# handasontam/PERT-GNN-KDD23

Measured on AMD Instinct MI355X. Metric: training graphs/sec (whole node), higher is better.
Workload: dtype bf16; 1 GPU; model=PERT-GNN 8L/256H, global_batch=1024, vocab=realistic, interfaces=2041, entry_unions=266, graph_mode=full, parallelism=dp1

## Files before the change

### csrc/bindings.cpp

```cpp
#include <hip/hip_runtime.h>
#include <torch/extension.h>

#include <climits>
#include <cstdlib>
#include <memory>
#include <optional>
#include <string>
#include <vector>

#include <c10/cuda/CUDAStream.h>

#include "hip/attn_bn.h"
#include "hip/gemm_dispatch.h"

namespace {

#define CHECK_IN(t)                                                      \
  TORCH_CHECK((t).is_cuda(), #t " must be on GPU");                      \
  TORCH_CHECK((t).is_contiguous(), #t " must be contiguous")

inline hipStream_t cur_stream() {
  return (hipStream_t)c10::cuda::getCurrentCUDAStream().stream();
}

// ... 143 lines not shown
                 float, float, float, float, hipStream_t);
void launch_adam_dynamic(float*, const float*, float*, float*, float*, float*,
                         long, float, float, float, float, float, float,
                         float, hipStream_t);
void launch_gemm_f32_nt(const float*, const float*, const float*, float*, int,
                        int, int, bool, hipStream_t);
void launch_gemm_f32_nn(const float*, const float*, const float*, float*, int,
                        int, int, bool, hipStream_t);
void launch_gemm_f32_tn(const float*, const float*, float*, float*, int, int,
                        int, hipStream_t);
void launch_colsum(const float*, float*, long, int, hipStream_t);
void launch_gemm_bf16_nt(const float*, const float*, const float*, float*,
                         int, int, int, bool, hipStream_t);
void launch_gemm_bf16_nn(const float*, const float*, const float*, float*,
                         int, int, int, bool, hipStream_t);
void launch_gemm_bf16_tn(const float*, const float*, float*, float*, int, int,
                         int, hipStream_t);
void launch_gemm_fp16_nt(const float*, const float*, const float*, float*,
                         int, int, int, bool, hipStream_t);
void launch_gemm_fp16_nn(const float*, const float*, const float*, float*,
                         int, int, int, bool, hipStream_t);
void launch_gemm_fp16_tn(const float*, const float*, float*, float*, int, int,
                         int, hipStream_t);
void launch_embed_grouped_scatter(const float*, const int*, const int*, float*,
                                  float*, long, int, int, int, int, int,
                                  hipStream_t);
void launch_embed_grouped_scatter_bal(const void*, int, const int*,
                                      const int*, const int*, const int*,
                                      const int*, const int*, float*, float*,
                                      float*, int, int, int, int, int, int,
                                      hipStream_t);
void launch_rows_sum_lists(const void*, int, const int*, const int*, void*, int,
                           int, int, int, hipStream_t);
void launch_vocab_scatter(const float*, const long*, long, float*, long, int,
                          int, int, int, hipStream_t);
void launch_vocab_scatter_dual(const float*, const long*, int, float*, float*,
                               long, int, int, int, hipStream_t);
void launch_edge_attn_fused_fwd(const float*, const float*, const float*,
                                const long*, int, const int*, const int*,
                                float*, float*, int, int, int, hipStream_t);
void launch_edge_attn_fused_bwd(const float*, const float*, const float*,
                                const float*, const long*, int, const float*,
                                const int*, const int*, const int*,
                                const int*, const int*, float*, float*,
                                float*, int, int, long, int, hipStream_t);
void launch_edge_attn_fused_fwd16(const void*, const void*, const void*,
                                  int, const long*, int, const int*,
                                  const int*, void*, int, float*, int, int,
                                  int, hipStream_t);
void launch_edge_attn_fused_bwd16(const void*, int, const void*,
                                  const void*, const void*, int, const long*,
                                  int, const float*, const int*, const int*,
                                  const int*, const int*, const int*, void*,
                                  void*, float*, int, int, long, int,
                                  hipStream_t, const AttnBnBwd* = nullptr,
                                  const AttnPoolBwd* = nullptr);
void launch_bn_bwd_partials_affine16(const void*, const void*,
                                     const unsigned char*, const float*,
                                     const float*, long, int, float*, float,
                                     float*, float*, float*, hipStream_t,
                                     bool acc = false);
void launch_edge_attn_fused_infer(const float*, const float*, const float*,
                                  const long*, int, const int*, const int*,
                                  const float*, const float*, int, float*,
                                  int, int, int, hipStream_t);
void launch_edge_attn_fused_infer16(const void*, const void*, const void*,
// ... 559 lines not shown
              "out_dtype must be bf16 or fp32");
  for (const auto& t : {idx1, lptr1, idx2, lptr2, idx3, lptr3})
    TORCH_CHECK(t.scalar_type() == torch::kInt32 && t.dim() == 1,
                "plan tensors must be 1-D int32");
  TORCH_CHECK(V >= 0 && R >= 0 && lptr3.numel() == V + R + 1,
              "lptr3 must have V+R+1 entries");
  TORCH_CHECK(lptr1.numel() >= 1 && lptr2.numel() >= 1,
              "lptr1/lptr2 must have at least one entry");
  TORCH_CHECK(idx1.numel() == de.size(0),
              "level 1 must list every row of de exactly once");
  const int h = (int)de.size(1);
  const long n1 = lptr1.numel() - 1;
  const long n2 = lptr2.numel() - 1;
  const int in16 = de.scalar_type() == torch::kBFloat16 ? 1 : 0;
  const int out16 = out_dtype == torch::kBFloat16 ? 1 : 0;
  auto partial =
      torch::empty({n1 + n2, (long)h}, de.options().dtype(torch::kFloat32));
  auto out = torch::empty({V + R, (long)h}, de.options().dtype(out_dtype));
  hipStream_t s = cur_stream();
  launch_rows_sum_lists(de.data_ptr(), in16, idx1.data_ptr<int>(),
                        lptr1.data_ptr<int>(), partial.data_ptr(), 0, (int)n1,
                        h, (int)unroll, s);
  if (n2 > 0)
    launch_rows_sum_lists(partial.data_ptr(), 0, idx2.data_ptr<int>(),
                          lptr2.data_ptr<int>(),
                          partial.data_ptr<float>() + n1 * h, 0, (int)n2, h,
                          (int)unroll, s);
  launch_rows_sum_lists(partial.data_ptr(), 0, idx3.data_ptr<int>(),
                        lptr3.data_ptr<int>(), out.data_ptr(), out16,
                        (int)(V + R), h, (int)unroll, s);
  return out;
}

std::vector<torch::Tensor> edge_attn_fused_fwd(
    torch::Tensor qkvs, torch::Tensor pifc, torch::Tensor prpc,
    torch::Tensor ea, torch::Tensor row_ptr, torch::Tensor csr_src,
    bool out16, int64_t heads = 1) {
  CHECK_IN(qkvs); CHECK_IN(pifc); CHECK_IN(prpc); CHECK_IN(ea);
  const int n = qkvs.size(0);
  const int h = qkvs.size(1) / 4;
  TORCH_CHECK(h <= 512, "H must be <= 512");
  TORCH_CHECK(heads >= 1 && heads <= h && h % heads == 0,
              "heads must divide H (H=", h, ", heads=", heads, ")");
  auto fopt = qkvs.options().dtype(torch::kFloat32);
  const bool b16 = qkvs.scalar_type() == torch::kBFloat16;
  const bool p16 = pifc.scalar_type() == torch::kBFloat16;
  TORCH_CHECK(!out16 || b16, "out16 requires bf16 qkvs");
  TORCH_CHECK(!p16 || b16, "bf16 P tables require bf16 qkvs");
  TORCH_CHECK(pifc.scalar_type() == prpc.scalar_type(),
              "P tables must share a dtype");
  auto out = torch::empty({n, h}, out16 ? qkvs.options() : fopt);
  auto alpha = heads == 1 ? torch::empty({ea.size(0)}, fopt)
                          : torch::empty({ea.size(0), heads}, fopt);
  if (b16) {
    launch_edge_attn_fused_fwd16(
        qkvs.data_ptr(), pifc.data_ptr(), prpc.data_ptr(), p16 ? 1 : 0,
        ea.data_ptr<long>(), (int)ea.size(1),
        row_ptr.data_ptr<int>(), csr_src.data_ptr<int>(),
        out.data_ptr(), out16 ? 1 : 0, alpha.data_ptr<float>(), n, h,
        (int)heads, cur_stream());
  } else {
    launch_edge_attn_fused_fwd(
        qkvs.data_ptr<float>(), pifc.data_ptr<float>(), prpc.data_ptr<float>(),
        ea.data_ptr<long>(), (int)ea.size(1), row_ptr.data_ptr<int>(),
        csr_src.data_ptr<int>(), out.data_ptr<float>(), alpha.data_ptr<float>(),
        n, h, (int)heads, cur_stream());
// ... 1087 lines not shown
                    sink_t[1] ? sink_t[1] : d_rpc.data_ptr<float>()};
  const int ms[2] = {(int)rows[0], (int)rows[1]};
  const bool addto[2] = {sink_t[0] != nullptr || splits > 1,
                         sink_t[1] != nullptr || splits > 1};
  launch_ptables_dgrad(dp_d.data(), w_d.data(), npairs, outs, ms, h, splits,
                       addto, s);
  launch_ptables_wgrad((int)dp_w.size(), dp_w.data(), a_w.data(), dw_w.data(),
                       m_w.data(), h, false, s, sunk.get());
  return {d_ifc, d_rpc, dW};
}

PYBIND11_MODULE(TORCH_EXTENSION_NAME, mod) {
  mod.def("ptables_fwd", &ptables_fwd, py::arg("ifc_table"),
          py::arg("rpc_table"), py::arg("we_ifc"), py::arg("we_rpc"));
  mod.def("ptables_bwd", &ptables_bwd, py::arg("dP"), py::arg("ifc_table"),
          py::arg("rpc_table"), py::arg("we_ifc"), py::arg("we_rpc"),
          py::arg("dgrad_splits") = 1, py::arg("d_ifc_sink") = py::none(),
          py::arg("d_rpc_sink") = py::none(),
          py::arg("dw_sinks") = std::vector<OptTensor>());
  mod.def("ptables_max_groups", &ptables_max_groups);
  mod.def("linear_fwd_bf16_o16", &linear_fwd_bf16_o16);
  mod.def("linear_dgrad16", &linear_dgrad16);
  mod.def("linear_wgrad16", &linear_wgrad16, py::arg("g"), py::arg("x"),
          py::arg("has_bias"), py::arg("dw_sink") = py::none(),
          py::arg("db_sink") = py::none(), py::arg("tile") = 0);
  mod.def("vocab_scatter_dual", &vocab_scatter_dual);
  mod.def("linear_dgrad", &linear_dgrad);
  mod.def("linear_wgrad", &linear_wgrad);
  mod.def("embed_grouped_scatter_bal", &embed_grouped_scatter_bal);
  mod.def("edge_table_grad", &edge_table_grad, py::arg("de"), py::arg("idx1"),
          py::arg("lptr1"), py::arg("idx2"), py::arg("lptr2"),
          py::arg("idx3"), py::arg("lptr3"), py::arg("V"), py::arg("R"),
          py::arg("out_dtype"), py::arg("unroll") = 8);
  mod.def("bn_stats", &bn_stats);
  mod.def("bn_finalize_apply", &bn_finalize_apply, py::arg("x"),
          py::arg("partials"), py::arg("gamma"), py::arg("beta"),
          py::arg("running_mean"), py::arg("running_var"), py::arg("momentum"),
          py::arg("eps"), py::arg("training"), py::arg("relu"),
          py::arg("dropout_p") = 0.0, py::arg("seed") = torch::Tensor());
  mod.def("bn_bwd_partials", &bn_bwd_partials, py::arg("g"), py::arg("x"),
          py::arg("y"), py::arg("mean"), py::arg("invstd"), py::arg("relu"),
          py::arg("keep_inv") = 1.0);
  mod.def("bn_bwd_apply", &bn_bwd_apply, py::arg("g"), py::arg("x"),
          py::arg("y"), py::arg("mean"), py::arg("invstd"), py::arg("gamma"),
          py::arg("partials_global"), py::arg("partials_local"),
          py::arg("relu"), py::arg("keep_inv") = 1.0,
          py::arg("dgamma_sink") = py::none(),
          py::arg("dbeta_sink") = py::none());
  mod.def("vocab_scatter", &vocab_scatter);
  mod.def("collate_native", &collate_native,
          py::call_guard<py::gil_scoped_release>());
  mod.def("edge_attn_fused_fwd", &edge_attn_fused_fwd, py::arg("qkvs"),
          py::arg("pifc"), py::arg("prpc"), py::arg("edge_attr"),
          py::arg("row_ptr"), py::arg("csr_src"), py::arg("out16"),
          py::arg("heads") = 1);
  mod.def("edge_attn_fused_bwd", &edge_attn_fused_bwd, py::arg("g"),
          py::arg("qkvs"), py::arg("pifc"), py::arg("prpc"),
          py::arg("edge_attr"), py::arg("alpha"), py::arg("row_ptr"),
          py::arg("csr_src"), py::arg("col_ptr"), py::arg("csc_dst"),
          py::arg("csc_eid"), py::arg("heads") = 1);
  mod.def("edge_attn_fused_infer", &edge_attn_fused_infer, py::arg("qkvs"),
          py::arg("pifc"), py::arg("prpc"), py::arg("edge_attr"),
          py::arg("row_ptr"), py::arg("csr_src"), py::arg("bn_scale"),
          py::arg("bn_shift"), py::arg("relu"), py::arg("out16"),
          py::arg("heads") = 1);
  mod.def("embed_grouped_scatter", &embed_grouped_scatter);
// ... 99 lines not shown
```

### csrc/hip/gemm.hip

```cpp

#include "common.h"
#include "gemm_dispatch.h"
#include <cstdlib>

static inline bool pertgnn_deterministic() {
  const char* e = getenv("PERTGNN_DETERMINISTIC");
  return e && e[0] == '1';
}

#define GEMM_BK 32
#define GEMM_THREADS 256

typedef __attribute__((ext_vector_type(4))) float f32x4;


template <int BF>
__device__ __forceinline__ void stage_transpose(
    const float* __restrict__ g, long ld, int free0, int contract0,
    int free_max, int contract_max, float* lds) {
  const int t = threadIdx.x;
  const int fr = t / 8;
  const int cq = (t % 8) * 4;
  const bool interior = (free0 + BF <= free_max) &&
                        (contract0 + GEMM_BK <= contract_max);
// ... 319 lines not shown
        a, b, bias, c, m, n, k2, relu ? 1 : 0);
  } else {
    const int grid = ((m + 63) / 64) * ((k2 + 63) / 64);
    gemm_f32_nn_kernel<64, 64><<<dim3(grid), dim3(GEMM_THREADS), 0, s>>>(
        a, b, bias, c, m, n, k2, relu ? 1 : 0);
  }
}

void launch_gemm_f32_tn(const float* a, const float* b, float* c, float* dbias,
                        int m, int n, int k2, hipStream_t s) {
  const bool big = gemm_dispatch::tn_tile128(n, k2);
  const int tiles = gemm_dispatch::tn_tiles(n, k2);
  const int slices =
      gemm_dispatch::tn_slices(m, tiles, GEMM_BK, pertgnn_deterministic());
  if (slices > 1)
    HIP_CHECK(hipMemsetAsync(c, 0, (long)n * k2 * sizeof(float), s));
  if (dbias) HIP_CHECK(hipMemsetAsync(dbias, 0, n * sizeof(float), s));
  if (big)
    gemm_f32_tn_kernel<128, 128>
        <<<dim3(tiles * slices), dim3(GEMM_THREADS), 0, s>>>(a, b, c, dbias, m,
                                                             n, k2, slices);
  else
    gemm_f32_tn_kernel<64, 64>
        <<<dim3(tiles * slices), dim3(GEMM_THREADS), 0, s>>>(a, b, c, dbias, m,
                                                             n, k2, slices);
}

void launch_colsum(const float* g, float* out, long m, int n, hipStream_t s) {
  HIP_CHECK(hipMemsetAsync(out, 0, n * sizeof(float), s));
  const int blocks = (int)min((long)256, (m + 63) / 64);
  colsum_par_kernel<<<dim3(blocks), dim3(256), n * sizeof(float), s>>>(g, out,
                                                                       m, n);
}
```

### csrc/hip/segops.hip

```cpp
#include "common.h"
#include <cstdlib>


#define WAVES_PER_BLOCK 4

template <int VPT, typename TX = float>
__global__ void seg_pool_p1_kernel(const TX* __restrict__ x,
                                   const float* __restrict__ probs,
                                   const float* __restrict__ nn,
                                   const int* __restrict__ batch_ptr,
                                   float* __restrict__ partial, int b, int P,
                                   int h) {
  const int wid = threadIdx.x / PERTGNN_WAVE;
  const int lane = threadIdx.x % PERTGNN_WAVE;
  const int w = blockIdx.x * WAVES_PER_BLOCK + wid;
  if (w >= b * P) return;
  const int g = w / P;
  const int sub = w % P;
  float acc[VPT];
#pragma unroll
  for (int j = 0; j < VPT; ++j) acc[j] = 0.f;
  for (int i = batch_ptr[g] + sub; i < batch_ptr[g + 1]; i += P) {
    const float wt = probs[i] / nn[i];
#pragma unroll
// ... 371 lines not shown
    embed_grouped_p2_kernel<V>                                                 \
        <<<dim3(ceil_div(rows, WAVES_PER_BLOCK)), block, 0, s>>>(              \
            partial, dtable, rows, P, h);                                      \
    break;
    CASE(1) CASE(2) CASE(3) CASE(4) CASE(5) CASE(6) CASE(7) CASE(8)
#undef CASE
    default: pertgnn_shape_fail("segops launcher", "vpt", vpt);
  }
}

template <int VPT, typename T>
__device__ __forceinline__ void rows_sum_load(const T* __restrict__ row,
                                              int lane, float (&v)[VPT]) {
  if constexpr (sizeof(T) == 2) {
#pragma unroll
    for (int q = 0; q < VPT; q += 4) {
      const segb4 x = *reinterpret_cast<const segb4*>(
          (const __bf16*)row + lane * VPT + q);
#pragma unroll
      for (int u = 0; u < 4; ++u) v[q + u] = (float)x[u];
    }
  } else {
#pragma unroll
    for (int q = 0; q < VPT; q += 4) {
      const segf4 x = *reinterpret_cast<const segf4*>(
          (const float*)row + lane * VPT + q);
#pragma unroll
      for (int u = 0; u < 4; ++u) v[q + u] = x[u];
    }
  }
}

template <int VPT, typename TIn, typename TOut, int U>
__global__ void rows_sum_lists_kernel(const TIn* __restrict__ src,
                                      const int* __restrict__ idx,
                                      const int* __restrict__ lptr,
                                      TOut* __restrict__ out, int n_lists) {
  static_assert(VPT % 4 == 0, "packed loads need 4 columns per lane");
  constexpr int H = VPT * PERTGNN_WAVE;
  const int lane = threadIdx.x % PERTGNN_WAVE;
  const int w = __builtin_amdgcn_readfirstlane(
      blockIdx.x * WAVES_PER_BLOCK + threadIdx.x / PERTGNN_WAVE);
  if (w >= n_lists) return;
  const int p0 = lptr[w];
  const int p1 = lptr[w + 1];
  float acc[VPT];
#pragma unroll
  for (int j = 0; j < VPT; ++j) acc[j] = 0.f;
  int p = p0;
  for (; p + U <= p1; p += U) {
    int r[U];
#pragma unroll
    for (int u = 0; u < U; ++u) r[u] = idx[p + u];
    float v[U][VPT];
#pragma unroll
    for (int u = 0; u < U; ++u)
      rows_sum_load<VPT>(src + (long)r[u] * H, lane, v[u]);
#pragma unroll
    for (int u = 0; u < U; ++u)
#pragma unroll
      for (int j = 0; j < VPT; ++j) acc[j] += v[u][j];
  }
  if (p < p1) {
    int r[U];
#pragma unroll
    for (int u = 0; u < U; ++u) r[u] = idx[min(p + u, p1 - 1)];
    float v[U][VPT];
#pragma unroll
    for (int u = 0; u < U; ++u)
      rows_sum_load<VPT>(src + (long)r[u] * H, lane, v[u]);
#pragma unroll
    for (int u = 0; u < U; ++u)
      if (p + u < p1) {
#pragma unroll
        for (int j = 0; j < VPT; ++j) acc[j] += v[u][j];
      }
  }
  TOut* dst = out + (long)w * H + lane * VPT;
  if constexpr (sizeof(TOut) == 2) {
#pragma unroll
    for (int q = 0; q < VPT; q += 4) {
      segb4 o;
#pragma unroll
      for (int u = 0; u < 4; ++u) o[u] = (__bf16)acc[q + u];
      *reinterpret_cast<segb4*>((__bf16*)dst + q) = o;
    }
  } else {
#pragma unroll
    for (int q = 0; q < VPT; q += 4) {
      segf4 o;
#pragma unroll
      for (int u = 0; u < 4; ++u) o[u] = acc[q + u];
      *reinterpret_cast<segf4*>((float*)dst + q) = o;
    }
  }
}

void launch_rows_sum_lists(const void* src, int in16, const int* idx,
                           const int* lptr, void* out, int out16, int n_lists,
                           int h, int unroll, hipStream_t s) {
  if (n_lists == 0) return;
  if (h != 256 && h != 512) pertgnn_shape_fail("rows_sum_lists", "h", h);
  if (unroll != 4 && unroll != 8)
    pertgnn_shape_fail("rows_sum_lists", "unroll", unroll);
  if (in16 && out16) pertgnn_shape_fail("rows_sum_lists", "in16+out16", 1);
  const dim3 block(WAVES_PER_BLOCK * PERTGNN_WAVE);
  const dim3 grid(ceil_div(n_lists, WAVES_PER_BLOCK));
#define RSL(V, TI, TO, UU)                                                     \
  rows_sum_lists_kernel<V, TI, TO, UU><<<grid, block, 0, s>>>(                 \
      (const TI*)src, idx, lptr, (TO*)out, n_lists)
#define RSL_T(V, UU)                                                           \
  do {                                                                         \
    if (in16) RSL(V, __bf16, float, UU);                                       \
    else if (out16) RSL(V, float, __bf16, UU);                                 \
    else RSL(V, float, float, UU);                                             \
  } while (0)
  if (h == 256) {
    if (unroll == 8) RSL_T(4, 8); else RSL_T(4, 4);
  } else {
    if (unroll == 8) RSL_T(8, 8); else RSL_T(8, 4);
  }
#undef RSL_T
#undef RSL
}

__global__ void vocab_scatter_kernel(const float* __restrict__ g,
                                     const long* __restrict__ idx,
                                     long idx_stride, float* __restrict__ dtable,
                                     long n, int rows, int h, int gstride,
                                     int col_off) {
  extern __shared__ float acc[];
  const long vh = (long)rows * h;
  for (long t = threadIdx.x; t < vh; t += blockDim.x) acc[t] = 0.f;
  __syncthreads();
  const int wid = threadIdx.x / PERTGNN_WAVE;
  const int lane = threadIdx.x % PERTGNN_WAVE;
  const long rows_per_block = (n + gridDim.x - 1) / gridDim.x;
  const long r0 = (long)blockIdx.x * rows_per_block;
  const long r1 = min(n, r0 + rows_per_block);
  for (long r = r0 + wid; r < r1; r += WAVES_PER_BLOCK) {
    const long v = idx[r * idx_stride];
    for (int c = lane; c < h; c += PERTGNN_WAVE)
      atomicAdd(&acc[v * h + c], g[r * gstride + col_off + c]);
  }
  __syncthreads();
  for (long t = threadIdx.x; t < vh; t += blockDim.x)
    if (acc[t] != 0.f) atomicAdd(&dtable[t], acc[t]);
}

__global__ void vocab_scatter_vec_kernel(const float* __restrict__ g,
                                         const long* __restrict__ idx,
                                         long idx_stride,
                                         float* __restrict__ dtable, long n,
                                         int rows, int h, int gstride,
                                         int col_off) {
  typedef __attribute__((ext_vector_type(4))) float f4;
// ... 1775 lines not shown
```

### pertgnn/models/pert_gnn.py

```python
from __future__ import annotations

import torch
import torch.nn.functional as F
from torch import nn

from ..ops import functional as ops


class _EdgeLinearView:

    def __init__(self, conv):
        object.__setattr__(self, "_conv", conv)

    @property
    def weight(self):
        c = self._conv
        return torch.cat([c.we_ifc, c.we_rpc], dim=1)

    bias = None


class _SegLinearView:

    def __init__(self, conv, seg, has_bias=True):
# ... 123 lines not shown

    def forward_fused(self, x, edge_attr, ifc_weight, rpc_weight, csr,
                      out16=False, pifc=None, prpc=None):
        qkvs, pifc, prpc = self._fused_operands(x, ifc_weight, rpc_weight,
                                                pifc, prpc)
        return ops.edge_attention_fused(qkvs, pifc, prpc, edge_attr, csr,
                                        out16=out16, heads=self.heads)

    def forward_fused_bn(self, x, edge_attr, ifc_weight, rpc_weight, csr, bn,
                         comm=None, dropout_p=0.0, pifc=None, prpc=None):
        qkvs, pifc, prpc = self._fused_operands(x, ifc_weight, rpc_weight,
                                                pifc, prpc)
        return ops.edge_attention_fused_bn_relu(
            qkvs, pifc, prpc, edge_attr, csr, bn.weight, bn.bias,
            bn.running_mean, bn.running_var, bn.momentum, bn.eps,
            heads=self.heads, comm=comm, dropout_p=dropout_p)

    def forward_fused_pool(self, x, edge_attr, ifc_weight, rpc_weight, csr,
                           probs, nnodes, batch, num_graphs, pifc=None,
                           prpc=None):
        qkvs, pifc, prpc = self._fused_operands(x, ifc_weight, rpc_weight,
                                                pifc, prpc)
        return ops.edge_attention_fused_pool(
            qkvs, pifc, prpc, edge_attr, csr, probs, nnodes, batch,
            num_graphs, heads=self.heads)

    def _fused_operands(self, x, ifc_weight, rpc_weight, pifc, prpc):
        h = self.out_channels
        if x.shape[1] != self.k_padded:
            x = torch.nn.functional.pad(x, (0, self.k_padded - x.shape[1]))
        act16 = (ops.gemm_precision() in ("bf16", "fp16") and h % 256 == 0
                 and ops.act16_enabled())
        if act16:
            qkvs = ops.linear16(x, self.w4, self.b4)
            if pifc is not None and prpc is not None:
                pass
            elif ops.p16_enabled():
                pifc = ops.linear16(ifc_weight, self.we_ifc)
                prpc = ops.linear16(rpc_weight, self.we_rpc)
            else:
                pifc = ops.linear(ifc_weight, self.we_ifc, None)
                prpc = ops.linear(rpc_weight, self.we_rpc, None)
        else:
            qkvs = ops.linear(x, self.w4, self.b4)
            pifc = ops.linear(ifc_weight, self.we_ifc, None)
            prpc = ops.linear(rpc_weight, self.we_rpc, None)
        return qkvs, pifc, prpc


class SAGEDeterministic(nn.Module):

    def __init__(
        self,
        in_channels,
        cat_dims,
        entry_id_max,
        interface_id_max,
        rpctype_id_max,
        hidden_channels,
        num_layers,
        dropout,
        *,
        heads=1,
    ):
        super().__init__()
        self.heads = heads
        self.convs = nn.ModuleList()
# ... 140 lines not shown
```

### pertgnn/ops/functional.py

```python
from __future__ import annotations

from typing import NamedTuple

import torch

from . import reference as ref
from .backend import ext, use_hip


def deterministic() -> bool:
    import os
    return os.environ.get("PERTGNN_DETERMINISTIC", "0") == "1"


def grad_sink(p):
    sink = getattr(p, "_grad_sink", None)
    if sink is None or not p.requires_grad or not torch.is_grad_enabled():
        return None
    import os
    if os.environ.get("PERTGNN_NO_GRAD_SINK", "0") == "1":
        return None
    g = p.grad
    if g is None or g.data_ptr() != sink.data_ptr() or g.shape != sink.shape:
        return None
# ... 160 lines not shown
    assert idx3.numel() == 0 or int(idx3.max()) < n1 + n2
    assert max(E, n1 + n2, idx3.numel(), idx2.numel()) < 2 ** 31
    i32 = lambda t: t.to(torch.int32)
    return EdgeTablePlan(i32(order), i32(lptr1), i32(idx2), i32(lptr2),
                         i32(idx3), i32(lptr3), n1, n2, V, R, C)


def edge_table_plan(edge_attr: torch.Tensor, V: int, R: int,
                    C: int | None = None) -> EdgeTablePlan:
    if C is None:
        C = _scatter_iters()
    key = ("edge_table", edge_attr.data_ptr(), edge_attr.numel(),
           tuple(edge_attr.stride()), V, R, C)
    hit = _GROUP_CACHE.get(key)
    if hit is not None:
        _GROUP_CACHE.move_to_end(key)
        return hit[1]
    ea = edge_attr[:, :2].cpu().long()
    plan = _build_edge_table_plan(ea[:, 0].contiguous(), ea[:, 1].contiguous(),
                                  V, R, C)
    dev = edge_attr.device
    plan = plan._replace(**{f: getattr(plan, f).to(dev) for f in
                            ("idx1", "lptr1", "idx2", "lptr2", "idx3",
                             "lptr3")})
    nbytes = sum(t.numel() for t in plan.tensors()) * 4
    while _GROUP_CACHE and _GROUP_CACHE_BYTES[0] + nbytes > _GROUP_CACHE_CAP:
        _, old = _GROUP_CACHE.popitem(last=False)
        _GROUP_CACHE_BYTES[0] -= old[-1]
    _GROUP_CACHE[key] = (edge_attr, plan, nbytes)
    _GROUP_CACHE_BYTES[0] += nbytes
    return plan


def apply_plan_reference(plan: EdgeTablePlan, de: torch.Tensor):
    acc = torch.float64 if de.dtype == torch.float64 else torch.float32
    h = de.shape[1]

    def level(src, idx, lptr):
        lens = (lptr[1:] - lptr[:-1]).long()
        seg = torch.repeat_interleave(
            torch.arange(lens.numel(), device=src.device), lens)
        out = torch.zeros(lens.numel(), h, dtype=acc, device=src.device)
        return out.index_add_(0, seg, src.index_select(0, idx.long()))

    p1 = level(de.to(acc), plan.idx1, plan.lptr1)
    p2 = level(p1, plan.idx2, plan.lptr2)
    out = level(torch.cat([p1, p2]), plan.idx3, plan.lptr3)
    return out[:plan.V], out[plan.V:]


def _edge_table_grads(m, de, pifc, prpc, edge_attr):
    V, R, h = pifc.shape[0], prpc.shape[0], de.shape[1]
    if h in (256, 512) and (V * h * 4 > 160 * 1024 or deterministic()):
        if de.dtype not in (torch.float32, torch.bfloat16):
            de = de.float()
        plan = edge_table_plan(edge_attr, V, R)
        od = pifc.dtype if pifc.dtype == torch.bfloat16 else torch.float32
        out = m.edge_table_grad(de, *plan.tensors(), V, R, od).to(pifc.dtype)
        return out[:V], out[V:]
    dpifc = _table_grad(m, de, edge_attr[:, 0], V, h, 0)
    dprpc = _table_grad(m, de, edge_attr[:, 1], R, h, 0)
    if dpifc.dtype != pifc.dtype:
        dpifc = dpifc.to(pifc.dtype)
        dprpc = dprpc.to(prpc.dtype)
    return dpifc, dprpc

# ... 77 lines not shown
            y = m.linear_fwd_bf16_o16(x, w, bb)
        ctx.save_for_backward(x, w)
        ctx.has_bias = b is not None
        ctx.fp16c = fp16c
        return y

    @staticmethod
    def backward(ctx, g):
        x, w = ctx.saved_tensors
        m = ext()
        g = g.contiguous()
        if x.dtype == torch.bfloat16:
            dx = m.linear_dgrad16_o16(g, w, ctx.fp16c, ctx.wt16)
            dw, db = m.linear_wgrad16_b16(g, x, ctx.has_bias, ctx.fp16c,
                                          ctx.w_sink, ctx.b_sink)
        else:
            dx = m.linear_dgrad16(g, w)
            dw, db = m.linear_wgrad16(g, x, ctx.has_bias, ctx.w_sink,
                                      ctx.b_sink)
        if ctx.w_sink is not None:
            return dx, None, None, None, None, None
        return dx, dw, (db if ctx.has_bias else None), None, None, None


def linear16(x, w, b=None):
    w_sink = grad_sink(w)
    b_sink = grad_sink(b) if b is not None else None
    if w_sink is None or (b is not None and b_sink is None):
        w_sink = b_sink = None
    if w_sink is None:
        return _Linear16Fn.apply(x, w, b)
    return _Linear16Fn.apply(x, _sunk(w, w_sink), _sunk(b, b_sink), w_sink,
                             b_sink, _sink_anchor(x.device))


class _PTablesFn(torch.autograd.Function):

    @staticmethod
    def forward(ctx, sinks, anchor, ifc_table, rpc_table, *weights):
        layers = len(weights) // 2
        we_ifc, we_rpc = list(weights[:layers]), list(weights[layers:])
        ctx.sinks = sinks
        ctx.set_materialize_grads(False)
        ctx.save_for_backward(ifc_table, rpc_table, *weights)
        return tuple(ext().ptables_fwd(ifc_table, rpc_table, we_ifc, we_rpc))

    @staticmethod
    def backward(ctx, *dps):
        ifc_table, rpc_table, *weights = ctx.saved_tensors
        layers = len(weights) // 2
        none = torch.empty(0, dtype=torch.bfloat16, device=ifc_table.device)
        t_sinks, w_sinks = ctx.sinks[:2], list(ctx.sinks[2:])
        d_ifc, d_rpc, dw = ext().ptables_bwd(
            [none if g is None else g.contiguous() for g in dps],
            ifc_table, rpc_table, weights[:layers], weights[layers:],
            ptable_dgrad_splits(), t_sinks[0], t_sinks[1], w_sinks)
        slot, dws = 0, []
        for g, sink in zip(dps, w_sinks):
            dws.append(None if g is None or sink is not None else dw[slot])
            slot += sink is None
        return (None, None,
                None if t_sinks[0] is not None else d_ifc,
                None if t_sinks[1] is not None else d_rpc, *dws)


def ptables_grouped(ifc_table, rpc_table, we_ifc, we_rpc):
# ... 188 lines not shown
        dx_raw = None
        if ctx.needs_input_grad[0]:
            dx_raw = g[:, : ctx.f].contiguous()
            if dx_raw.dtype != torch.float32:
                dx_raw = dx_raw.float()
        dtable = None
        if ctx.needs_input_grad[2]:
            dtable = _table_grad(m, g, cat_idx, ctx.rows, ctx.h, ctx.f)
        return dx_raw, None, dtable, None, None


class _EmbedEdgeFn(torch.autograd.Function):
    @staticmethod
    def forward(ctx, edge_attr, ifc_table, rpc_table):
        m = ext()
        out = m.embed_edge_fwd(edge_attr, ifc_table, rpc_table)
        ctx.save_for_backward(edge_attr)
        ctx.rows = (ifc_table.shape[0], rpc_table.shape[0])
        return out

    @staticmethod
    def backward(ctx, g):
        (edge_attr,) = ctx.saved_tensors
        m = ext()
        g = g.contiguous()
        h = g.shape[1] // 2
        d_ifc = _table_grad(m, g, edge_attr[:, 0], ctx.rows[0], h, 0)
        d_rpc = _table_grad(m, g, edge_attr[:, 1], ctx.rows[1], h, h)
        return None, d_ifc, d_rpc


def embed_concat_node(x_raw, cat_X, tables, out16=False, pad_to=None):
    if len(tables) == 1 and use_hip(x_raw):
        return _EmbedNodeFn.apply(x_raw, cat_X[:, 0].contiguous(), tables[0],
                                  out16, 0 if pad_to is None else int(pad_to))
    out = ref.embed_concat_node(x_raw, cat_X, tables)
    if pad_to is not None:
        if pad_to < out.shape[1]:
            raise ValueError(f"pad_to={pad_to} is below the concat width "
                             f"{out.shape[1]}")
        out = torch.nn.functional.pad(out, (0, pad_to - out.shape[1]))
    return out


def embed_concat_edge(edge_attr, interface_table, rpctype_table):
    if use_hip(interface_table):
        return _EmbedEdgeFn.apply(edge_attr, interface_table, rpctype_table)
    return ref.embed_concat_edge(edge_attr, interface_table, rpctype_table)



class _EmbeddingFn(torch.autograd.Function):
    @staticmethod
    def forward(ctx, idx, table):
        m = ext()
        out = m.gather_rows(idx, table)
        ctx.save_for_backward(idx)
        ctx.rows = table.shape[0]
        return out

    @staticmethod
    def backward(ctx, g):
        (idx,) = ctx.saved_tensors
        m = ext()
        g = g.contiguous()
        return None, _table_grad(m, g, idx, ctx.rows, g.shape[1], 0)


# ... 439 lines not shown
```

Measured before the change: 124,200 graphs/s.

## Fold embedding-table gradient through first linear layer's backward

Replaces the input gradient of the first linear layer plus the embedding scatter with a fused path. The bf16 output gradient is first summed per category index using a multi-level segment-sum plan. A small fp32 GEMM against the table's slice of the weight then yields the table gradient directly, so the full dx GEMM over every node is skipped. This adds a cached CPU-built plan per category index tensor, and relies on attaching metadata to the embedding output tensor and detaching x, so gradients to x are dropped.

```diff
diff --git a/csrc/bindings.cpp b/csrc/bindings.cpp
--- a/csrc/bindings.cpp
+++ b/csrc/bindings.cpp
@@ -199,6 +199,10 @@
                                       hipStream_t);
 void launch_rows_sum_lists(const void*, int, const int*, const int*, void*, int,
                            int, int, int, hipStream_t);
+void launch_rows_sum_lists_wide(const void*, int, int, const int*, const int*,
+                                float*, int, int, int, int, int, hipStream_t);
+void launch_embed_fold_gemm(const float*, const float*, float*, int, int, int,
+                            int, int, bool, hipStream_t);
 void launch_vocab_scatter(const float*, const long*, long, float*, long, int,
                           int, int, int, hipStream_t);
 void launch_vocab_scatter_dual(const float*, const long*, int, float*, float*,
@@ -824,6 +828,62 @@
   return out;
 }
 
+torch::Tensor embed_dgrad_fold(torch::Tensor dqkvs, torch::Tensor idx1,
+                               torch::Tensor lptr1, torch::Tensor idx2,
+                               torch::Tensor lptr2, torch::Tensor idx3,
+                               torch::Tensor lptr3, torch::Tensor w4,
+                               int64_t f, int64_t h, int64_t rows,
+                               OptTensor sink = std::nullopt,
+                               int64_t unroll = 8, int64_t seg_cols = 256) {
+  CHECK_IN(dqkvs); CHECK_IN(idx1); CHECK_IN(lptr1); CHECK_IN(idx2);
+  CHECK_IN(lptr2); CHECK_IN(idx3); CHECK_IN(lptr3); CHECK_IN(w4);
+  TORCH_CHECK(h == 256 || h == 512, "embed_dgrad_fold: h must be 256 or 512");
+  TORCH_CHECK(dqkvs.dim() == 2 && dqkvs.size(1) == 4 * h &&
+                  dqkvs.scalar_type() == torch::kBFloat16,
+              "embed_dgrad_fold: dqkvs must be bf16 [n, 4h]");
+  TORCH_CHECK(w4.dim() == 2 && w4.size(0) == 4 * h &&
+                  w4.scalar_type() == torch::kFloat32,
+              "embed_dgrad_fold: w4 must be fp32 [4h, k_padded]");
+  TORCH_CHECK(f >= 0 && f + h <= w4.size(1),
+              "embed_dgrad_fold: columns f..f+h must lie inside w4");
+  for (const auto& t : {idx1, lptr1, idx2, lptr2, idx3, lptr3})
+    TORCH_CHECK(t.scalar_type() == torch::kInt32 && t.dim() == 1,
+                "plan tensors must be 1-D int32");
+  TORCH_CHECK(rows >= 0 && lptr3.numel() == rows + 1,
+              "embed_dgrad_fold: lptr3 must have rows+1 entries");
+  TORCH_CHECK(lptr1.numel() >= 1 && lptr2.numel() >= 1,
+              "lptr1/lptr2 must have at least one entry");
+  TORCH_CHECK(idx1.numel() == dqkvs.size(0),
+              "level 1 must list every row of dqkvs exactly once");
+  float* sink_p = grad_sink(sink, dqkvs, {rows, h}, "embed_dgrad_fold");
+  auto fopt = dqkvs.options().dtype(torch::kFloat32);
+  if (dqkvs.size(0) == 0 || rows == 0)
+    return sink_p ? torch::empty({0}, fopt) : torch::zeros({rows, h}, fopt);
+  const int width = (int)(4 * h);
+  const long n1 = lptr1.numel() - 1;
+  const long n2 = lptr2.numel() - 1;
+  auto buf = torch::empty({n1 + n2 + rows, (long)width}, fopt);
+  float* p = buf.data_ptr<float>();
+  float* G = p + (n1 + n2) * width;
+  hipStream_t s = cur_stream();
+  launch_rows_sum_lists_wide(dqkvs.data_ptr(), 1, width, idx1.data_ptr<int>(),
+                             lptr1.data_ptr<int>(), p, width, (int)n1, width,
+                             (int)seg_cols, (int)unroll, s);
+  if (n2 > 0)
+    launch_rows_sum_lists_wide(p, 0, width, idx2.data_ptr<int>(),
+                               lptr2.data_ptr<int>(), p + n1 * width, width,
+                               (int)n2, width, (int)seg_cols, (int)unroll, s);
+  launch_rows_sum_lists_wide(p, 0, width, idx3.data_ptr<int>(),
+                             lptr3.data_ptr<int>(), G, width, (int)rows, width,
+                             (int)seg_cols, (int)unroll, s);
+  auto out = torch::empty({sink_p ? 0 : rows, sink_p ? 0 : h}, fopt);
+  launch_embed_fold_gemm(G, w4.data_ptr<float>(),
+                         sink_p ? sink_p : out.data_ptr<float>(), (int)rows,
+                         width, (int)h, (int)w4.size(1), (int)f,
+                         sink_p != nullptr, s);
+  return out;
+}
+
 std::vector<torch::Tensor> edge_attn_fused_fwd(
     torch::Tensor qkvs, torch::Tensor pifc, torch::Tensor prpc,
     torch::Tensor ea, torch::Tensor row_ptr, torch::Tensor csr_src,
@@ -1977,6 +2037,11 @@
           py::arg("lptr1"), py::arg("idx2"), py::arg("lptr2"),
           py::arg("idx3"), py::arg("lptr3"), py::arg("V"), py::arg("R"),
           py::arg("out_dtype"), py::arg("unroll") = 8);
+  mod.def("embed_dgrad_fold", &embed_dgrad_fold, py::arg("dqkvs"),
+          py::arg("idx1"), py::arg("lptr1"), py::arg("idx2"), py::arg("lptr2"),
+          py::arg("idx3"), py::arg("lptr3"), py::arg("w4"), py::arg("f"),
+          py::arg("h"), py::arg("rows"), py::arg("sink") = py::none(),
+          py::arg("unroll") = 8, py::arg("seg_cols") = 256);
   mod.def("bn_stats", &bn_stats);
   mod.def("bn_finalize_apply", &bn_finalize_apply, py::arg("x"),
           py::arg("partials"), py::arg("gamma"), py::arg("beta"),
diff --git a/csrc/hip/gemm.hip b/csrc/hip/gemm.hip
--- a/csrc/hip/gemm.hip
+++ b/csrc/hip/gemm.hip
@@ -375,3 +375,95 @@
   colsum_par_kernel<<<dim3(blocks), dim3(256), n * sizeof(float), s>>>(g, out,
                                                                        m, n);
 }
+
+#define EDF_BM 32
+#define EDF_BN 64
+#define EDF_BK 128
+
+template <bool ACC>
+__global__ __launch_bounds__(256) void embed_fold_gemm_kernel(
+    const float* __restrict__ G, const float* __restrict__ w,
+    float* __restrict__ out, int rows, int K, int h, int ldw, int col0) {
+  __shared__ float gs[EDF_BK][EDF_BM + 4];
+  __shared__ float bs[EDF_BK][EDF_BN];
+  const int t = threadIdx.x;
+  const int c0 = blockIdx.x * EDF_BN;
+  const int r0 = blockIdx.y * EDF_BM;
+  const int g_row = t / 8, g_kq = (t % 8) * 4;
+  const bool g_ok = r0 + g_row < rows;
+  const float* g_src = G + (long)(r0 + g_row) * K + g_kq;
+  const int b_c = t % EDF_BN, b_k = t / EDF_BN;
+  const float* b_src = w + (long)b_k * ldw + col0 + c0 + b_c;
+  const int tx = t % 16, ty = t / 16;
+
+  f32x4 g_reg[EDF_BK / 32];
+  float b_reg[EDF_BK / 4];
+  auto load = [&](int k0) {
+#pragma unroll
+    for (int i = 0; i < EDF_BK / 32; ++i)
+      g_reg[i] = g_ok ? *reinterpret_cast<const f32x4*>(g_src + k0 + 32 * i)
+                      : f32x4{0.f, 0.f, 0.f, 0.f};
+#pragma unroll
+    for (int i = 0; i < EDF_BK / 4; ++i)
+      b_reg[i] = (float)(__bf16)b_src[(long)(k0 + 4 * i) * ldw];
+  };
+  auto store = [&]() {
+#pragma unroll
+    for (int i = 0; i < EDF_BK / 32; ++i)
+#pragma unroll
+      for (int u = 0; u < 4; ++u) gs[g_kq + 32 * i + u][g_row] = g_reg[i][u];
+#pragma unroll
+    for (int i = 0; i < EDF_BK / 4; ++i) bs[b_k + 4 * i][b_c] = b_reg[i];
+  };
+
+  float acc[2][4];
+#pragma unroll
+  for (int i = 0; i < 2; ++i)
+#pragma unroll
+    for (int j = 0; j < 4; ++j) acc[i][j] = 0.f;
+
+  const int nk = K / EDF_BK;
+  load(0);
+  for (int kt = 0; kt < nk; ++kt) {
+    store();
+    __syncthreads();
+    if (kt + 1 < nk) load((kt + 1) * EDF_BK);
+#pragma unroll 8
+    for (int k = 0; k < EDF_BK; ++k) {
+      const float a0 = gs[k][ty * 2];
+      const float a1 = gs[k][ty * 2 + 1];
+      const f32x4 b = *reinterpret_cast<const f32x4*>(&bs[k][tx * 4]);
+#pragma unroll
+      for (int j = 0; j < 4; ++j) {
+        acc[0][j] = __builtin_fmaf(a0, b[j], acc[0][j]);
+        acc[1][j] = __builtin_fmaf(a1, b[j], acc[1][j]);
+      }
+    }
+    __syncthreads();
+  }
+#pragma unroll
+  for (int i = 0; i < 2; ++i) {
+    const int r = r0 + ty * 2 + i;
+    if (r >= rows) continue;
+    float* o = out + (long)r * h + c0 + tx * 4;
+#pragma unroll
+    for (int j = 0; j < 4; ++j) o[j] = ACC ? o[j] + acc[i][j] : acc[i][j];
+  }
+}
+
+void launch_embed_fold_gemm(const float* G, const float* w, float* out,
+                            int rows, int K, int h, int ldw, int col0,
+                            bool accumulate, hipStream_t s) {
+  if (rows == 0) return;
+  if (K <= 0 || K % EDF_BK != 0) pertgnn_shape_fail("embed_fold_gemm", "K", K);
+  if (h <= 0 || h % EDF_BN != 0) pertgnn_shape_fail("embed_fold_gemm", "h", h);
+  if (col0 < 0 || col0 + h > ldw)
+    pertgnn_shape_fail("embed_fold_gemm", "col0+h", (long)col0 + h);
+  const dim3 grid(h / EDF_BN, ceil_div(rows, EDF_BM));
+  if (accumulate)
+    embed_fold_gemm_kernel<true><<<grid, dim3(256), 0, s>>>(G, w, out, rows, K,
+                                                            h, ldw, col0);
+  else
+    embed_fold_gemm_kernel<false><<<grid, dim3(256), 0, s>>>(G, w, out, rows,
+                                                             K, h, ldw, col0);
+}
diff --git a/csrc/hip/segops.hip b/csrc/hip/segops.hip
--- a/csrc/hip/segops.hip
+++ b/csrc/hip/segops.hip
@@ -427,12 +427,11 @@
 }
 
 template <int VPT, typename TIn, typename TOut, int U>
-__global__ void rows_sum_lists_kernel(const TIn* __restrict__ src,
-                                      const int* __restrict__ idx,
-                                      const int* __restrict__ lptr,
-                                      TOut* __restrict__ out, int n_lists) {
+__device__ __forceinline__ void rows_sum_lists_body(
+    const TIn* __restrict__ src, const int* __restrict__ idx,
+    const int* __restrict__ lptr, TOut* __restrict__ out, int n_lists,
+    long src_stride, long out_stride) {
   static_assert(VPT % 4 == 0, "packed loads need 4 columns per lane");
-  constexpr int H = VPT * PERTGNN_WAVE;
   const int lane = threadIdx.x % PERTGNN_WAVE;
   const int w = __builtin_amdgcn_readfirstlane(
       blockIdx.x * WAVES_PER_BLOCK + threadIdx.x / PERTGNN_WAVE);
@@ -450,7 +449,7 @@
     float v[U][VPT];
 #pragma unroll
     for (int u = 0; u < U; ++u)
-      rows_sum_load<VPT>(src + (long)r[u] * H, lane, v[u]);
+      rows_sum_load<VPT>(src + (long)r[u] * src_stride, lane, v[u]);
 #pragma unroll
     for (int u = 0; u < U; ++u)
 #pragma unroll
@@ -463,7 +462,7 @@
     float v[U][VPT];
 #pragma unroll
     for (int u = 0; u < U; ++u)
-      rows_sum_load<VPT>(src + (long)r[u] * H, lane, v[u]);
+      rows_sum_load<VPT>(src + (long)r[u] * src_stride, lane, v[u]);
 #pragma unroll
     for (int u = 0; u < U; ++u)
       if (p + u < p1) {
@@ -471,7 +470,7 @@
         for (int j = 0; j < VPT; ++j) acc[j] += v[u][j];
       }
   }
-  TOut* dst = out + (long)w * H + lane * VPT;
+  TOut* dst = out + (long)w * out_stride + lane * VPT;
   if constexpr (sizeof(TOut) == 2) {
 #pragma unroll
     for (int q = 0; q < VPT; q += 4) {
@@ -489,6 +488,27 @@
       *reinterpret_cast<segf4*>((float*)dst + q) = o;
     }
   }
+}
+
+template <int VPT, typename TIn, typename TOut, int U>
+__global__ void rows_sum_lists_kernel(const TIn* __restrict__ src,
+                                      const int* __restrict__ idx,
+                                      const int* __restrict__ lptr,
+                                      TOut* __restrict__ out, int n_lists) {
+  constexpr int H = VPT * PERTGNN_WAVE;
+  rows_sum_lists_body<VPT, TIn, TOut, U>(src, idx, lptr, out, n_lists, H, H);
+}
+
+template <int VPT, typename TIn, int U>
+__global__ void rows_sum_lists_wide_kernel(const TIn* __restrict__ src,
+                                           const int* __restrict__ idx,
+                                           const int* __restrict__ lptr,
+                                           float* __restrict__ out,
+                                           int n_lists, int src_stride,
+                                           int out_stride) {
+  const int col0 = blockIdx.y * (VPT * PERTGNN_WAVE);
+  rows_sum_lists_body<VPT, TIn, float, U>(src + col0, idx, lptr, out + col0,
+                                          n_lists, src_stride, out_stride);
 }
 
 void launch_rows_sum_lists(const void* src, int in16, const int* idx,
@@ -517,6 +537,40 @@
   }
 #undef RSL_T
 #undef RSL
+}
+
+void launch_rows_sum_lists_wide(const void* src, int in16, int src_stride,
+                                const int* idx, const int* lptr, float* out,
+                                int out_stride, int n_lists, int width,
+                                int seg_cols, int unroll, hipStream_t s) {
+  if (n_lists == 0) return;
+  if (seg_cols != 256 && seg_cols != 512)
+    pertgnn_shape_fail("rows_sum_lists_wide", "seg_cols", seg_cols);
+  if (width <= 0 || width % seg_cols != 0)
+    pertgnn_shape_fail("rows_sum_lists_wide", "width", width);
+  if (src_stride < width || out_stride < width || src_stride % 4 != 0 ||
+      out_stride % 4 != 0)
+    pertgnn_shape_fail("rows_sum_lists_wide", "stride",
+                       src_stride < out_stride ? src_stride : out_stride);
+  if (unroll != 4 && unroll != 8)
+    pertgnn_shape_fail("rows_sum_lists_wide", "unroll", unroll);
+  const dim3 block(WAVES_PER_BLOCK * PERTGNN_WAVE);
+  const dim3 grid(ceil_div(n_lists, WAVES_PER_BLOCK), width / seg_cols);
+#define RSW(V, TI, UU)                                                         \
+  rows_sum_lists_wide_kernel<V, TI, UU><<<grid, block, 0, s>>>(                \
+      (const TI*)src, idx, lptr, out, n_lists, src_stride, out_stride)
+#define RSW_T(V, UU)                                                           \
+  do {                                                                         \
+    if (in16) RSW(V, __bf16, UU);                                              \
+    else RSW(V, float, UU);                                                    \
+  } while (0)
+  if (seg_cols == 256) {
+    if (unroll == 8) RSW_T(4, 8); else RSW_T(4, 4);
+  } else {
+    if (unroll == 8) RSW_T(8, 8); else RSW_T(8, 4);
+  }
+#undef RSW_T
+#undef RSW
 }
 
 __global__ void vocab_scatter_kernel(const float* __restrict__ g,
diff --git a/pertgnn/models/pert_gnn.py b/pertgnn/models/pert_gnn.py
--- a/pertgnn/models/pert_gnn.py
+++ b/pertgnn/models/pert_gnn.py
@@ -179,7 +179,7 @@
         act16 = (ops.gemm_precision() in ("bf16", "fp16") and h % 256 == 0
                  and ops.act16_enabled())
         if act16:
-            qkvs = ops.linear16(x, self.w4, self.b4)
+            qkvs = ops.linear16_embed(x, self.w4, self.b4)
             if pifc is not None and prpc is not None:
                 pass
             elif ops.p16_enabled():
diff --git a/pertgnn/ops/functional.py b/pertgnn/ops/functional.py
--- a/pertgnn/ops/functional.py
+++ b/pertgnn/ops/functional.py
@@ -216,6 +216,61 @@
     return plan
 
 
+def _build_cat_table_plan(idx, rows: int, C: int):
+    n = idx.numel()
+    if n and (int(idx.min()) < 0 or int(idx.max()) >= rows):
+        raise IndexError("category index outside the embedding table")
+    order = torch.argsort(idx, stable=True)
+    counts = torch.bincount(idx, minlength=rows)
+    out_of_member, lptr1 = _chunk_segments(counts, C)
+    n1 = out_of_member.numel()
+    members = torch.arange(n1)
+    cnt = (counts + C - 1) // C
+    big = cnt > C
+    in_big = big[out_of_member]
+    idx2 = members[in_big]
+    _, lptr2 = _chunk_segments(cnt[big], C)
+    n2 = lptr2.numel() - 1
+    len3 = torch.where(big, (cnt + C - 1) // C, cnt)
+    lptr3 = torch.cat([torch.zeros(1, dtype=torch.long), len3.cumsum(0)])
+    from_l2 = big[torch.repeat_interleave(torch.arange(rows), len3)]
+    idx3 = torch.empty(int(len3.sum()), dtype=torch.long)
+    idx3[from_l2] = n1 + torch.arange(n2)
+    idx3[~from_l2] = members[~in_big]
+    assert order.numel() == n and int(lptr1[-1]) == n
+    assert int(lptr2[-1]) == idx2.numel() and int(lptr3[-1]) == idx3.numel()
+    assert idx2.numel() == 0 or int(idx2.max()) < n1
+    assert idx3.numel() == 0 or int(idx3.max()) < n1 + n2
+    assert max(n, n1 + n2, idx3.numel(), idx2.numel()) < 2 ** 31
+    i32 = lambda t: t.to(torch.int32)
+    return EdgeTablePlan(i32(order), i32(lptr1), i32(idx2), i32(lptr2),
+                         i32(idx3), i32(lptr3), n1, n2, rows, 0, C)
+
+
+def cat_table_plan(cat_idx: torch.Tensor, rows: int,
+                   C: int | None = None) -> EdgeTablePlan:
+    if C is None:
+        C = _scatter_iters()
+    key = ("cat_table", cat_idx.data_ptr(), cat_idx.numel(),
+           tuple(cat_idx.stride()), rows, C)
+    hit = _GROUP_CACHE.get(key)
+    if hit is not None:
+        _GROUP_CACHE.move_to_end(key)
+        return hit[1]
+    plan = _build_cat_table_plan(cat_idx.cpu().long().contiguous(), rows, C)
+    dev = cat_idx.device
+    plan = plan._replace(**{f: getattr(plan, f).to(dev) for f in
+                            ("idx1", "lptr1", "idx2", "lptr2", "idx3",
+                             "lptr3")})
+    nbytes = sum(t.numel() for t in plan.tensors()) * 4
+    while _GROUP_CACHE and _GROUP_CACHE_BYTES[0] + nbytes > _GROUP_CACHE_CAP:
+        _, old = _GROUP_CACHE.popitem(last=False)
+        _GROUP_CACHE_BYTES[0] -= old[-1]
+    _GROUP_CACHE[key] = (cat_idx, plan, nbytes)
+    _GROUP_CACHE_BYTES[0] += nbytes
+    return plan
+
+
 def apply_plan_reference(plan: EdgeTablePlan, de: torch.Tensor):
     acc = torch.float64 if de.dtype == torch.float64 else torch.float32
     h = de.shape[1]
@@ -359,6 +414,74 @@
         return _Linear16Fn.apply(x, w, b)
     return _Linear16Fn.apply(x, _sunk(w, w_sink), _sunk(b, b_sink), w_sink,
                              b_sink, _sink_anchor(x.device))
+
+
+def embed_dgrad_fold_enabled() -> bool:
+    import os
+    return os.environ.get("PERTGNN_NO_EMBED_DGRAD_FOLD", "0") != "1"
+
+
+class EmbedSource(NamedTuple):
+    cat_idx: torch.Tensor
+    table: torch.Tensor
+    f: int
+    h: int
+    x_raw_requires_grad: bool
+
+
+class _Linear16EmbedFn(torch.autograd.Function):
+
+    @staticmethod
+    def forward(ctx, x, w, b, table, cat_idx, f, w_sink, b_sink, t_sink,
+                anchor):
+        m = ext()
+        bb = b if b is not None else torch.empty(0, dtype=torch.float32, device=x.device)
+        ctx.w_sink, ctx.b_sink, ctx.t_sink = w_sink, b_sink, t_sink
+        y = m.linear_fwd_a16o16(x, w, bb, False)
+        ctx.save_for_backward(x, w, cat_idx)
+        ctx.has_bias = b is not None
+        ctx.f, ctx.rows, ctx.h = f, table.shape[0], table.shape[1]
+        return y
+
+    @staticmethod
+    def backward(ctx, g):
+        x, w, cat_idx = ctx.saved_tensors
+        m = ext()
+        g = g.contiguous()
+        dw, db = m.linear_wgrad16_b16(g, x, ctx.has_bias, False, ctx.w_sink,
+                                      ctx.b_sink)
+        dtable = None
+        if ctx.t_sink is not None or ctx.needs_input_grad[3]:
+            plan = cat_table_plan(cat_idx, ctx.rows)
+            dtable = m.embed_dgrad_fold(g, *plan.tensors(), w, ctx.f, ctx.h,
+                                        ctx.rows, ctx.t_sink)
+            if ctx.t_sink is not None:
+                dtable = None
+        if ctx.w_sink is not None:
+            dw = db = None
+        return (None, dw, (db if ctx.has_bias else None), dtable, None, None,
+                None, None, None, None)
+
+
+def linear16_embed(x, w, b=None):
+    src = getattr(x, "_embed_src", None)
+    if (src is None or not embed_dgrad_fold_enabled()
+            or not torch.is_grad_enabled()
+            or x.dtype != torch.bfloat16 or gemm_precision() != "bf16"
+            or src.x_raw_requires_grad or src.h not in (256, 512)
+            or not src.table.requires_grad or not x.requires_grad
+            or w.shape[0] != 4 * src.h or src.f + src.h > w.shape[1]
+            or x.shape[1] != w.shape[1]):
+        return linear16(x, w, b)
+    w_sink = grad_sink(w)
+    b_sink = grad_sink(b) if b is not None else None
+    if w_sink is None or (b is not None and b_sink is None):
+        w_sink = b_sink = None
+    t_sink = grad_sink(src.table)
+    return _Linear16EmbedFn.apply(
+        x.detach(), _sunk(w, w_sink), _sunk(b, b_sink),
+        _sunk(src.table, t_sink), src.cat_idx, src.f, w_sink, b_sink, t_sink,
+        _sink_anchor(x.device))
 
 
 class _PTablesFn(torch.autograd.Function):
@@ -613,8 +736,12 @@
 
 def embed_concat_node(x_raw, cat_X, tables, out16=False, pad_to=None):
     if len(tables) == 1 and use_hip(x_raw):
-        return _EmbedNodeFn.apply(x_raw, cat_X[:, 0].contiguous(), tables[0],
-                                  out16, 0 if pad_to is None else int(pad_to))
+        cat_idx = cat_X[:, 0]
+        out = _EmbedNodeFn.apply(x_raw, cat_idx.contiguous(), tables[0],
+                                 out16, 0 if pad_to is None else int(pad_to))
+        out._embed_src = EmbedSource(cat_idx, tables[0], x_raw.shape[1],
+                                     tables[0].shape[1], x_raw.requires_grad)
+        return out
     out = ref.embed_concat_node(x_raw, cat_X, tables)
     if pad_to is not None:
         if pad_to < out.shape[1]:
```

Measured after the change: 128,400 graphs/s, median of 6. 1.03x the previous value.
